# clberube/BISIP

Measured on AMD Instinct MI355X. Metric: log-prob evals/sec (walker-steps/s), PolynomialDecomposition 32 freq fp64, higher is better.
Workload: dtype f64; 1 GPU; PolynomialDecomposition poly_deg=5 c_exp=1.0, 32 synthetic frequencies (S=64 taus), ndim 7, theta uniform in the prior box; walkers_per_gpu=16777216, global_walkers=16777216, parallelism=walker-sharded x1, no data-path collective, kernel=k_logprob_pd_reduced, variant=reduced

## Files before the change

bisip_amd/_hip.py:

```python

import ctypes
import importlib.util
import os
import sys

import numpy as np

_HERE = os.path.dirname(os.path.abspath(__file__))
LIB_PATH = os.path.join(_HERE, 'libbisip_hip.so')

MODEL_POLYDECOMP, MODEL_COLECOLE, MODEL_DIAS2000, MODEL_SHIN2015 = 0, 1, 2, 3
VARIANT_AUTO, VARIANT_FAITHFUL, VARIANT_COLLAPSED, VARIANT_REDUCED, VARIANT_WAVE, VARIANT_REDUCED_COMP = 0, 1, 2, 3, 4, 5
VARIANTS = {'auto': VARIANT_AUTO, 'faithful': VARIANT_FAITHFUL, 'collapsed': VARIANT_COLLAPSED,
            'reduced': VARIANT_REDUCED, 'wave': VARIANT_WAVE, 'reduced_comp': VARIANT_REDUCED_COMP}

_dp = ctypes.POINTER(ctypes.c_double)


class ModelDesc(ctypes.Structure):
    _fields_ = [('n_modes', ctypes.c_int), ('poly_deg', ctypes.c_int), ('n_taus', ctypes.c_int),
                ('c_exp', ctypes.c_double), ('taus', _dp), ('log_taus', _dp)]


class StretchArgs(ctypes.Structure):
# ... 25 lines not shown
                                          ctypes.POINTER(ModelDesc)]),
    'bisip_ctx_nspectra': (ctypes.c_int, [ctypes.c_void_p]),
    'bisip_ctx_destroy': (None, [ctypes.c_void_p]),
    'bisip_ctx_set_bounds': (ctypes.c_int, [ctypes.c_void_p, _dp, _dp]),
    'bisip_ctx_set_spectrum_offset': (ctypes.c_int, [ctypes.c_void_p, ctypes.c_int64]),
    'bisip_ctx_set_variant': (ctypes.c_int, [ctypes.c_void_p, ctypes.c_int]),
    'bisip_ctx_get_variant': (ctypes.c_int, [ctypes.c_void_p]),
    'bisip_logprob': (ctypes.c_int, [ctypes.c_void_p, _dp, ctypes.c_int64, _dp]),
    'bisip_logprob_dev': (ctypes.c_int, [ctypes.c_void_p, ctypes.c_void_p, ctypes.c_int64,
                                         ctypes.c_void_p, ctypes.c_void_p]),
    'bisip_forward': (ctypes.c_int, [ctypes.c_void_p, _dp, ctypes.c_int64, _dp]),
    'bisip_forward_dev': (ctypes.c_int, [ctypes.c_void_p, ctypes.c_void_p, ctypes.c_int64,
                                         ctypes.c_void_p, ctypes.c_void_p]),
    'bisip_loglike_z': (ctypes.c_int, [ctypes.c_void_p, _dp, ctypes.c_int64, _dp]),
    'bisip_loglike_z_dev': (ctypes.c_int, [ctypes.c_void_p, ctypes.c_void_p, ctypes.c_int64,
                                           ctypes.c_void_p, ctypes.c_void_p]),
    'bisip_stretch_half_dev': (ctypes.c_int, [ctypes.c_void_p, ctypes.POINTER(StretchArgs), ctypes.c_void_p]),
    'bisip_stretch_eval_dev': (ctypes.c_int, [ctypes.c_void_p, ctypes.POINTER(StretchArgs), ctypes.c_void_p]),
    'bisip_stretch_apply_dev': (ctypes.c_int, [ctypes.c_void_p, ctypes.POINTER(StretchArgs), ctypes.c_void_p]),
    'bisip_stretch_run_dev': (ctypes.c_int, [ctypes.c_void_p, ctypes.POINTER(StretchArgs), ctypes.c_int64,
                                             ctypes.c_int64, ctypes.c_int64, ctypes.c_void_p]),
    'bisip_stretch_run_sharded_dev': (ctypes.c_int, [ctypes.c_void_p, ctypes.c_void_p, ctypes.POINTER(StretchArgs),
                                                     ctypes.c_int64, ctypes.c_int64, ctypes.c_int64, ctypes.c_void_p]),
    'bisip_stretch_run_sharded_sim_dev': (ctypes.c_int, [ctypes.c_void_p, ctypes.c_int, ctypes.POINTER(StretchArgs),
                                                         ctypes.c_int64, ctypes.c_int64, ctypes.c_int64, ctypes.c_void_p]),
    'bisip_rccl_unique_id': (ctypes.c_int, [ctypes.c_void_p]),
    'bisip_rccl_comm_create': (ctypes.c_int, [ctypes.POINTER(ctypes.c_void_p), ctypes.c_int, ctypes.c_int,
                                              ctypes.c_void_p, ctypes.c_int]),
    'bisip_rccl_comm_destroy': (ctypes.c_int, [ctypes.c_void_p]),
    'bisip_stretch_draw_dev': (ctypes.c_int, [ctypes.c_void_p, ctypes.c_int64, ctypes.c_double,
                                              ctypes.c_uint64, ctypes.c_int64, ctypes.c_int64] +
                               [ctypes.c_void_p] * 7),
    'bisip_stretch_philox_inline': (ctypes.c_int, [ctypes.c_void_p, ctypes.c_int64]),
    'bisip_stretch_run_philox_dev': (ctypes.c_int, [ctypes.c_void_p, ctypes.POINTER(StretchArgs), ctypes.c_int64, ctypes.c_int64,
                                                    ctypes.c_int64, ctypes.c_double, ctypes.c_uint64, ctypes.c_int64,
                                                    ctypes.c_void_p, ctypes.c_void_p]),
    'bisip_stretch_persistent_dev': (ctypes.c_int, [ctypes.c_void_p, ctypes.POINTER(PersistArgs), ctypes.c_void_p]),
    'bisip_chain_moments_workspace': (ctypes.c_int64, [ctypes.c_int64, ctypes.c_int64, ctypes.c_int]),
    'bisip_chain_moments_dev': (ctypes.c_int, [ctypes.c_void_p, ctypes.c_int64, ctypes.c_int64, ctypes.c_int64,
                                               ctypes.c_int64, ctypes.c_int] + [ctypes.c_void_p] * 4),
    'bisip_chain_percentiles_workspace': (ctypes.c_int64, [ctypes.c_int64, ctypes.c_int64, ctypes.c_int64, ctypes.c_int,
                                                           ctypes.c_int]),
    'bisip_chain_percentiles_dev': (ctypes.c_int, [ctypes.c_void_p, ctypes.c_int64, ctypes.c_int64, ctypes.c_int64,
                                                   ctypes.c_int64, ctypes.c_int, _dp, ctypes.c_int, ctypes.c_void_p,
                                                   ctypes.c_void_p, ctypes.c_int64, ctypes.c_void_p]),
    'bisip_chain_autocorr_time_workspace': (ctypes.c_int64, [ctypes.c_int64, ctypes.c_int64, ctypes.c_int64, ctypes.c_int]),
    'bisip_chain_autocorr_time_dev': (ctypes.c_int, [ctypes.c_void_p, ctypes.c_int64, ctypes.c_int64, ctypes.c_int64,
                                                     ctypes.c_int64, ctypes.c_int, ctypes.c_double] + [ctypes.c_void_p] * 4),
    'bisip_rtd_integrals_dev': (ctypes.c_int, [ctypes.c_void_p, ctypes.c_int64, ctypes.c_int64, ctypes.c_int64,
                                               ctypes.c_int64, ctypes.c_int] + [ctypes.c_void_p] * 4),
    'bisip_rtd_columns_dev': (ctypes.c_int, [ctypes.c_void_p, ctypes.c_int64, ctypes.c_int64, ctypes.c_int64,
                                             ctypes.c_int64, ctypes.c_int, ctypes.c_int64, ctypes.c_int64,
                                             ctypes.c_void_p, ctypes.c_int, ctypes.c_void_p, ctypes.c_void_p]),
    'bisip_chain_range_dev': (ctypes.c_int, [ctypes.c_void_p, ctypes.c_int64, ctypes.c_int64, ctypes.c_int64,
                                             ctypes.c_int64, ctypes.c_int] + [ctypes.c_void_p] * 3),
    'bisip_chain_histograms_dev': (ctypes.c_int, [ctypes.c_void_p, ctypes.c_int64, ctypes.c_int64, ctypes.c_int64,
                                                  ctypes.c_int64, ctypes.c_int, ctypes.c_void_p, ctypes.c_int,
                                                  ctypes.c_void_p, ctypes.c_void_p]),
    'bisip_chain_pair_histograms_dev': (ctypes.c_int, [ctypes.c_void_p, ctypes.c_int64, ctypes.c_int64, ctypes.c_int64,
                                                       ctypes.c_int64, ctypes.c_int, ctypes.c_void_p, ctypes.c_int,
                                                       ctypes.c_void_p, ctypes.c_void_p]),
    'bisip_chain_trace_workspace': (ctypes.c_int64, [ctypes.c_int64, ctypes.c_int64, ctypes.c_int64, ctypes.c_int, ctypes.c_int]),
    'bisip_chain_trace_lds_walkers': (ctypes.c_int, [ctypes.c_int]),
    'bisip_chain_trace_dev': (ctypes.c_int, [ctypes.c_void_p, ctypes.c_int64, ctypes.c_int64, ctypes.c_int64, ctypes.c_int64,
                                             ctypes.c_int, _dp, ctypes.c_int, ctypes.c_void_p, ctypes.c_void_p, ctypes.c_void_p,
                                             ctypes.c_int64, ctypes.c_void_p]),
# ... 419 lines not shown
                                                   int(W), ctypes.c_void_p(d_Z_ptr), ctypes.c_void_p(stream)))

    def stretch_half_dev(self, args, stream=0):
        _check(self._lib.bisip_stretch_half_dev(self._h, ctypes.byref(args), ctypes.c_void_p(stream)))

    def stretch_eval_dev(self, args, stream=0):
        _check(self._lib.bisip_stretch_eval_dev(self._h, ctypes.byref(args), ctypes.c_void_p(stream)))

    def stretch_apply_dev(self, args, stream=0):
        _check(self._lib.bisip_stretch_apply_dev(self._h, ctypes.byref(args), ctypes.c_void_p(stream)))

    def stretch_run_dev(self, first_args, W, n_steps, thin_by=1, stream=0):
        _check(self._lib.bisip_stretch_run_dev(self._h, ctypes.byref(first_args), int(W),
                                               int(n_steps), int(thin_by), ctypes.c_void_p(stream)))

    def stretch_run_sharded_dev(self, comm, first_args, W, n_steps, thin_by=1, stream=0):
        _check(self._lib.bisip_stretch_run_sharded_dev(self._h, ctypes.c_void_p(comm), ctypes.byref(first_args),
                                                       int(W), int(n_steps), int(thin_by), ctypes.c_void_p(stream)))

    def stretch_run_sharded_sim_dev(self, world, first_args, W, n_steps, thin_by=1, stream=0):
        _check(self._lib.bisip_stretch_run_sharded_sim_dev(self._h, int(world), ctypes.byref(first_args),
                                                           int(W), int(n_steps), int(thin_by), ctypes.c_void_p(stream)))

    def stretch_persistent_dev(self, args, stream=0):
        rc = self._lib.bisip_stretch_persistent_dev(self._h, ctypes.byref(args), ctypes.c_void_p(stream))
        if rc == -4:
            return False
        _check(rc)
        return True

    def stretch_philox_inline(self, W):
        return bool(self._lib.bisip_stretch_philox_inline(self._h, int(W)))

    def stretch_run_philox_dev(self, first_args, W, n_steps, thin_by, a, seed, step0, perm, stream=0):
        _check(self._lib.bisip_stretch_run_philox_dev(self._h, ctypes.byref(first_args), int(W), int(n_steps), int(thin_by),
                                                      float(a), int(seed), int(step0), ctypes.c_void_p(perm),
                                                      ctypes.c_void_p(stream)))

    def stretch_draw_dev(self, W, a, seed, step0, n_steps, perm, active, partner, zz, factor, logu,
                         stream=0):
        _check(self._lib.bisip_stretch_draw_dev(self._h, int(W), float(a), int(seed), int(step0),
                                                int(n_steps), *[ctypes.c_void_p(p) for p in
                                                                (perm, active, partner, zz, factor, logu)],
                                                ctypes.c_void_p(stream)))


RCCL_ID_BYTES = 128


def clock_probe_dev(d_out_ptr, window_us, stream=0):
    _check(load_library().bisip_clock_probe_dev(ctypes.c_void_p(d_out_ptr), float(window_us), ctypes.c_void_p(stream)))


def fp64_stream_probe_lanes():
    return int(load_library().bisip_fp64_stream_probe_lanes())


def fp64_stream_probe_dev(d_out_ptr, rounds, stream=0):
    n = ctypes.c_int64(0)
    _check(load_library().bisip_fp64_stream_probe_dev(ctypes.c_void_p(d_out_ptr), int(rounds), ctypes.byref(n), ctypes.c_void_p(stream)))
    return int(n.value)


def rccl_unique_id():
    buf = ctypes.create_string_buffer(RCCL_ID_BYTES)
    _check(load_library().bisip_rccl_unique_id(buf))
# ... 229 lines not shown
```

bisip_amd/csrc/bisip_hip.hip:

```cpp
#include <cstdlib>

#include "host.h"
#include "host_precompute.h"
#include "chain_kernels.h"

#include <atomic>
#include <exception>

using namespace bisip;
using namespace bisip::host;

namespace {
thread_local char g_err[512] = "";
}

namespace bisip {
namespace host {

int fail(int code, const char *fmt, ...)
{
    va_list ap;
    va_start(ap, fmt);
    vsnprintf(g_err, sizeof(g_err), fmt, ap);
    va_end(ap);
// ... 903 lines not shown
}

int bisip_stretch_eval_dev(bisip_ctx *c, const bisip_stretch_args *u, void *stream)
{
    int rc = check_stretch(c, u, true);
    if (rc != BISIP_OK || u->n_slots == 0) return rc;
    if (!u->partner || !u->zz || !u->factor || !u->logu) return fail(BISIP_EINVAL, "null RNG stream");
    if (u->slot_lo < 0 || u->slot_hi > u->n_slots || u->slot_lo > u->slot_hi)
        return fail(BISIP_EINVAL, "bad slot range [%lld,%lld) of %lld", (long long)u->slot_lo,
                    (long long)u->slot_hi, (long long)u->n_slots);
    if (u->slot_lo == u->slot_hi) return BISIP_OK;
    HIP_TRY(hipSetDevice(c->device));
    const StretchArgs a = to_device_args(u);
    return dispatch_stretch(c, StretchWork{STRETCH_EVAL, &a, nullptr}, u->walkers_per_spectrum, (hipStream_t)stream);
}

int bisip_stretch_apply_dev(bisip_ctx *c, const bisip_stretch_args *u, void *stream)
{
    int rc = check_stretch(c, u, true);
    if (rc != BISIP_OK || u->n_slots == 0) return rc;
    if (u->world < 1 || u->pad * u->world < u->n_slots)
        return fail(BISIP_EINVAL, "gathered block too small: world=%d pad=%lld n_slots=%lld", u->world,
                    (long long)u->pad, (long long)u->n_slots);
    HIP_TRY(hipSetDevice(c->device));
    return dispatch_apply(c, to_device_args(u), (hipStream_t)stream);
}

static bool packed_state(const bisip_ctx *c, int64_t W, int64_t n_steps)
{
    return c->E == 1 && c->ndim < PACKED_ROW && W / 2 >= 65536 && lanes_per_walker(W / 2) == 1 && n_steps > 0 &&
           std::getenv("BISIP_NO_PACKED_STATE") == nullptr;
}

struct PhiloxStream {
    double a;
    uint64_t seed;
    int64_t step0;
    const int32_t *d_perm;
};

static int stretch_run(bisip_ctx *c, const bisip_stretch_args *first, int64_t W, int64_t n_steps, int64_t thin_by,
                       const PhiloxStream *draw, void *stream)
{
    const int64_t nh = (W + 1) / 2;
    bisip_stretch_args u = *first;
    const bool packed = packed_state(c, W, n_steps);
    if (draw && !packed) return fail(BISIP_EUNSUPPORTED, "the stream is drawn in place only by the packed-state half-step (bisip_stretch_philox_inline)");
    if (packed) {
        const size_t need = (size_t)W * PACKED_ROW * sizeof(double);
        if (c->packed_bytes < need) {
            if (c->d_packed) { HIP_TRY(hipDeviceSynchronize()); (void)hipFree(c->d_packed); c->d_packed = nullptr; c->packed_bytes = 0; }
            hipError_t e = hipMalloc((void **)&c->d_packed, need);
            if (e != hipSuccess) return fail(BISIP_ENOMEM, "hipMalloc(%zu) failed: %s", need, hipGetErrorString(e));
            c->packed_bytes = need;
        }
        hipLaunchKernelGGL(k_state_repack<true>, dim3((unsigned)((W + 255) / 256)), dim3(256), 0, (hipStream_t)stream,
                           first->coords, first->logp, c->d_packed, (long long)W, c->ndim);
        HIP_TRY(hipGetLastError());
    }
    for (int64_t k = 0; k < n_steps; ++k) {
        for (int h = 0; h < 2; ++h) {
            const int64_t off = (k * 2 + h) * nh;
            if (!draw) {
                u.active = first->active + off; u.partner = first->partner + off;
                u.zz = first->zz + off; u.factor = first->factor + off; u.logu = first->logu + off;
            }
            u.n_slots = h ? W / 2 : nh;
            const bool store = ((k + 1) % thin_by) == 0;
            const int64_t srow = k / thin_by;
            u.chain_row = (store && first->chain_row) ? first->chain_row + srow * W * c->ndim : nullptr;
            u.logp_row = (store && first->logp_row) ? first->logp_row + srow * W : nullptr;
            StretchArgs a = to_device_args(&u);
            if (packed) a.packed = c->d_packed;
            if (draw) {
                a.perm = draw->d_perm + 3 * k;
                a.draw_W = W; a.draw_a = draw->a; a.draw_ndim_m1 = (double)(c->ndim - 1);
                a.seed_lo = (unsigned int)(draw->seed & 0xffffffffu); a.seed_hi = (unsigned int)(draw->seed >> 32);
                a.draw_step = (unsigned int)(draw->step0 + k); a.draw_e = (unsigned int)c->spectrum_offset; a.draw_h = h;
            }
            int rc = dispatch_stretch(c, StretchWork{STRETCH_HALF, &a, nullptr}, u.walkers_per_spectrum, (hipStream_t)stream);
            if (rc != BISIP_OK) return rc;
        }
    }
    if (packed) {
        hipLaunchKernelGGL(k_state_repack<false>, dim3((unsigned)((W + 255) / 256)), dim3(256), 0, (hipStream_t)stream,
                           first->coords, first->logp, c->d_packed, (long long)W, c->ndim);
        HIP_TRY(hipGetLastError());
    }
    return BISIP_OK;
}

int bisip_stretch_run_dev(bisip_ctx *c, const bisip_stretch_args *first, int64_t W, int64_t n_steps,
                          int64_t thin_by, void *stream)
{
    if (!c || !first) return fail(BISIP_EINVAL, "null argument");
    if (thin_by < 1 || n_steps % thin_by) return fail(BISIP_EINVAL, "n_steps=%lld must be a multiple of thin_by=%lld", (long long)n_steps, (long long)thin_by);
    if (W < 2 || n_steps < 0) return fail(BISIP_EINVAL, "bad W=%lld or n_steps=%lld", (long long)W, (long long)n_steps);
    if (!first->coords || !first->logp || !first->active || !first->partner || !first->zz ||
        !first->factor || !first->logu || !first->status)
        return fail(BISIP_EINVAL, "null buffer");
    HIP_TRY(hipSetDevice(c->device));
    return stretch_run(c, first, W, n_steps, thin_by, nullptr, stream);
}

int bisip_stretch_philox_inline(const bisip_ctx *c, int64_t W)
{
    return c && W >= 2 && W <= 0x7fffffffLL && packed_state(c, W, 1) ? 1 : 0;
}

int bisip_stretch_run_philox_dev(bisip_ctx *c, const bisip_stretch_args *first, int64_t W, int64_t n_steps,
                                 int64_t thin_by, double a, uint64_t seed, int64_t step0, const int32_t *d_perm,
                                 void *stream)
{
    if (!c || !first || !d_perm) return fail(BISIP_EINVAL, "null argument");
    if (thin_by < 1 || n_steps % thin_by) return fail(BISIP_EINVAL, "n_steps=%lld must be a multiple of thin_by=%lld", (long long)n_steps, (long long)thin_by);
    if (W < 2 || W > 0x7fffffffLL || n_steps < 0 || step0 < 0 || step0 + n_steps > 0xffffffffLL)
        return fail(BISIP_EINVAL, "bad W=%lld or step range [%lld, +%lld)", (long long)W, (long long)step0, (long long)n_steps);
    if (!(a > 0.0)) return fail(BISIP_EINVAL, "stretch scale a=%g must be positive", a);
    if (!first->coords || !first->logp || !first->status) return fail(BISIP_EINVAL, "null buffer");
    if (n_steps == 0) return BISIP_OK;
    HIP_TRY(hipSetDevice(c->device));
    const PhiloxStream draw{a, seed, step0, d_perm};
    return stretch_run(c, first, W, n_steps, thin_by, &draw, stream);
}

static double reduced_check_rows(const bisip_ctx *c, const double *theta, int64_t W, const double *logp,
                                 int64_t lo, int64_t hi, int64_t stride)
{
    constexpr int BLOCK = 64;
    const int64_t per = c->E > 1 ? W / c->E : W;
    const int n = c->ndim;
    double rows[BLOCK * MAXD], want[BLOCK], got[BLOCK];
    int held = 0;
    int64_t spectrum = -1;
    double w = 0.0;
    auto flush = [&] {
        if (!held) return;
        reduced_logp_reference_rows(c->reduced[(size_t)spectrum], rows, held, want);
        for (int r = 0; r < held; ++r) {
            const double scale = std::fabs(want[r]) > 1.0 ? std::fabs(want[r]) : 1.0;
// ... 361 lines not shown
```

bisip_amd/csrc/dispatch_stretch.hip:

```cpp
#include "stretch_launch.h"

using namespace bisip;
using namespace bisip::host;

namespace {

template <class M>
int stretch_generic(const bisip_ctx *c, const StretchWork &a, hipStream_t st)
{
    const ModelOperands o{c->d_cb_lp ? c->d_cb_lp : c->d_cb, c->N, c->lconst};
    if constexpr (CoopLimit<M>::value > 0) {
        switch (stretch_lanes(a)) {
        case 8: { GenericLP<M, 8> lp; lp.o = o; lp.b = c->bounds; return launch_stretch(a, lp, st); }
        case 4: { GenericLP<M, 4> lp; lp.o = o; lp.b = c->bounds; return launch_stretch(a, lp, st); }
        case 2: { GenericLP<M, 2> lp; lp.o = o; lp.b = c->bounds; return launch_stretch(a, lp, st); }
        default: break;
        }
    }
    GenericLP<M, 1> lp; lp.o = o; lp.b = c->bounds;
    return launch_stretch(a, lp, st);
}

template <int P, bool COMP>
int stretch_reduced(const bisip_ctx *c, const StretchWork &a, hipStream_t st)
{
    ReducedLP<P, COMP> lp;
    fill_reduced<P, COMP>(c, lp.r);
    lp.lconst = c->lconst;
    lp.b = c->bounds;
    return launch_stretch(a, lp, st);
}

}

namespace bisip {
namespace host {

StretchArgs to_device_args(const bisip_stretch_args *u)
{
    StretchArgs a;
    a.coords = u->coords; a.logp = u->logp;
    a.active = u->active; a.partner = u->partner;
    a.zz = u->zz; a.factor = u->factor; a.logu = u->logu;
    a.n_slots = u->n_slots; a.slot_lo = u->slot_lo; a.slot_hi = u->slot_hi;
    a.block = u->block; a.chain_row = u->chain_row; a.logp_row = u->logp_row;
    a.naccept = u->naccept; a.status = u->status;
    a.pad = u->pad;
    a.packed = nullptr;
    a.perm = nullptr; a.draw_W = 0; a.draw_a = 0.0; a.draw_ndim_m1 = 0.0;
    a.seed_lo = a.seed_hi = a.draw_step = a.draw_e = 0u; a.draw_h = 0;
    const long long world = u->world > 0 ? u->world : 1;
    a.base = u->n_slots / world;
    a.extra = u->n_slots % world;
    return a;
}

int dispatch_stretch(const bisip_ctx *c, const StretchWork &a, long long Wp, hipStream_t st)
{
    if (c->E > 1) {
        if (Wp < 2 || (Wp & 1)) return fail(BISIP_EINVAL, "batch context: walkers_per_spectrum must be even and >= 2, got %lld", Wp);
        return dispatch_stretch_batch(c, a, Wp, st);
    }
    switch (c->model_id) {
    case BISIP_MODEL_POLYDECOMP:
        if (effective_variant(c) == BISIP_VARIANT_FAITHFUL || effective_variant(c) == BISIP_VARIANT_WAVE)
            return fail(BISIP_EUNSUPPORTED, "the device stretch move has no kernel for the faithful / wave "
                        "formulation: use variant auto, reduced or collapsed, or the host-loop sampler");
        if (effective_variant(c) == BISIP_VARIANT_REDUCED) {
            switch (c->P) {
#define X(p) case p: return stretch_reduced<p, false>(c, a, st);
                PD_CASES(X)
#undef X
            }
        } else if (effective_variant(c) == BISIP_VARIANT_REDUCED_COMP) {
            switch (c->P) {
#define X(p) case p: return stretch_reduced<p, true>(c, a, st);
                PD_CASES(X)
#undef X
            }
        } else {
            switch (c->P) {
#define X(p) case p: return stretch_generic<PDCollapsed<p>>(c, a, st);
// ... 34 lines not shown
```

bisip_amd/csrc/sampler_kernels.h:

```cpp
#pragma once
#include <type_traits>
#include "kernels.h"
#include "philox.h"

namespace bisip {

struct StretchArgs {
    double *coords;
    double *logp;
    const int *active;
    const int *partner;
    const double *zz;
    const double *factor;
    const double *logu;
    long long n_slots;
    long long slot_lo, slot_hi;
    double *block;
    double *chain_row;
    double *logp_row;
    int *naccept;
    int *status;
    long long pad, base, extra;
    double *packed;
    const int *perm;
    long long draw_W;
    double draw_a, draw_ndim_m1;
    unsigned int seed_lo, seed_hi, draw_step, draw_e;
    int draw_h;
};

template <class LP, class = void>
struct MayPersist : std::true_type {};
template <class LP>
struct MayPersist<LP, std::void_t<decltype(LP::WAVE_IN_ONE_SPECTRUM)>> : std::bool_constant<LP::WAVE_IN_ONE_SPECTRUM> {};

template <class LP, class = void>
struct SingleSpectrum : std::false_type {};
template <class LP>
struct SingleSpectrum<LP, std::void_t<decltype(LP::SINGLE_SPECTRUM)>> : std::bool_constant<LP::SINGLE_SPECTRUM> {};

template <class M, int L_ = 1>
struct GenericLP {
    static constexpr bool SINGLE_SPECTRUM = true;
    static constexpr int NDIM = M::NDIM;
    static constexpr int L = L_;
    static constexpr bool CAN_STAGE = true;
    static constexpr int REC_DOUBLES = M::REC;
    ModelOperands o;
    Bounds b;
    __device__ __forceinline__ double operator()(const double (&th)[NDIM], int, int g) const
    {
        return logprob_row<M, L>(th, o, b, g);
    }
    __device__ __forceinline__ const double *records(long long) const { return o.cb; }
    __host__ __device__ __forceinline__ int n_freq() const { return o.N; }
    struct Local {};
    __device__ __forceinline__ Local local(long long) const { return {}; }
// ... 223 lines not shown
                        a.zz[t], a.factor[t], a.logu[t], lp, i, g, a.status, row, lp_row);
}

template <int NDIM>
__device__ __forceinline__ void commit_row(const StretchArgs &a, int i, const double (&row)[NDIM],
                                           double lp_row, bool acc)
{
    if (acc) {
#pragma unroll
        for (int k = 0; k < NDIM; ++k) a.coords[(long long)i * NDIM + k] = row[k];
        a.logp[i] = lp_row;
    }
    if (a.chain_row) {
#pragma unroll
        for (int k = 0; k < NDIM; ++k) a.chain_row[(long long)i * NDIM + k] = row[k];
    }
    if (a.logp_row) a.logp_row[i] = lp_row;
    if (a.naccept && acc) atomicAdd(a.naccept + i, 1);
}

__device__ __forceinline__ int perm_inverse(long long y, long long W, long long Ainv, long long B)
{
    long long v = y - B;
    if (v < 0) v += W;
    if (W <= 65536) return (int)(((unsigned)Ainv * (unsigned)v) % (unsigned)W);
    const unsigned long long prod = (unsigned long long)Ainv * (unsigned long long)v;
    const unsigned q = (unsigned)((double)prod * (1.0 / (double)W));
    long long r = (long long)(prod - (unsigned long long)q * (unsigned long long)W);
    if (r < 0) r += W;
    if (r >= W) r -= W;
    return (int)r;
}

struct SlotDraw {
    int active, partner;
    double z, factor, logu;
};

__device__ __forceinline__ SlotDraw draw_slot(long long W, double a, double ndim_m1, unsigned seed_lo,
                                              unsigned seed_hi, unsigned step, int h, unsigned e,
                                              long long t, long long A_inv, long long B)
{
    const long long Nc = h ? (W + 1) / 2 : W / 2;
    const unsigned c2 = (unsigned)h | (e << 1);
    const Philox4 r0 = philox4x32_10((unsigned)t, step, c2, 0u, seed_lo, seed_hi);
    const Philox4 r1 = philox4x32_10((unsigned)t, step, c2, 1u, seed_lo, seed_hi);
    const double uz = u53(r0.v[0], r0.v[1]);
    const long long r = (long long)(((unsigned long long)r0.v[2] * (unsigned long long)Nc) >> 32);
    const double v = (a - 1.0) * uz + 1.0;
    SlotDraw d;
    d.z = (v * v) / a;
    d.active = perm_inverse(2 * t + h, W, A_inv, B);
    d.partner = perm_inverse(2 * r + (1 - h), W, A_inv, B);
    d.factor = ndim_m1 * log(d.z);
    d.logu = log(u53(r1.v[0], r1.v[1]));
    return d;
}

template <class LP, int BLK = 64>
__global__ __launch_bounds__(BLK) void k_stretch_half(const StretchArgs a, const LP lp)
{
    constexpr int L = LP::L;
    const long long tid = (long long)blockIdx.x * BLK + threadIdx.x;
    const long long slot = tid / L;
    const int g = (int)(tid % L);
    const bool live = slot < a.n_slots;
    const long long t = live ? slot : a.n_slots - 1;
    int i;
    double row[LP::NDIM], lp_row;
    const bool acc = stretch_slot(a, lp, t, g, i, row, lp_row);
    if (live && g == 0) commit_row<LP::NDIM>(a, i, row, lp_row, acc);
}

constexpr int PACKED_ROW = 8;

template <class LP, int BLK = 256>
__global__ __launch_bounds__(BLK) void k_stretch_half_packed(const StretchArgs a, const LP lp)
{
    static_assert(LP::L == 1 && LP::NDIM < PACKED_ROW, "one lane per slot, a walker in one 64-byte row");
    constexpr int NDIM = LP::NDIM;
    const long long slot = (long long)blockIdx.x * BLK + threadIdx.x;
    const bool live = slot < a.n_slots;
    const long long t = live ? slot : a.n_slots - 1;
    int i, p;
    double z, factor, logu;
    if (a.perm) {
        const SlotDraw d = draw_slot(a.draw_W, a.draw_a, a.draw_ndim_m1, a.seed_lo, a.seed_hi, a.draw_step, a.draw_h,
                                     a.draw_e, t, a.perm[1], a.perm[2]);
        i = d.active; p = d.partner; z = d.z; factor = d.factor; logu = d.logu;
    } else {
        i = __builtin_nontemporal_load(a.active + t); p = __builtin_nontemporal_load(a.partner + t);
    }
    const dbl2 *srow = reinterpret_cast<const dbl2 *>(a.packed + (long long)i * PACKED_ROW);
    const dbl2 *crow = reinterpret_cast<const dbl2 *>(a.packed + (long long)p * PACKED_ROW);
    dbl2 sv[4], cv[4];
#pragma unroll
    for (int q = 0; q < 4; ++q) { sv[q] = srow[q]; cv[q] = crow[q]; }
    if (!a.perm) {
        z = __builtin_nontemporal_load(a.zz + t); factor = __builtin_nontemporal_load(a.factor + t);
        logu = __builtin_nontemporal_load(a.logu + t);
    }
    double s_row[PACKED_ROW], c_row[PACKED_ROW];
#pragma unroll
    for (int q = 0; q < 4; ++q) { s_row[2 * q] = sv[q].x; s_row[2 * q + 1] = sv[q].y; c_row[2 * q] = cv[q].x; c_row[2 * q + 1] = cv[q].y; }
    double row[NDIM], lp_row;
    const bool acc = stretch_move(s_row, c_row, s_row[PACKED_ROW - 1], z, factor, logu, lp, i, 0, a.status, row, lp_row);
    if (!live) return;
    if (acc) {
        double r[PACKED_ROW];
#pragma unroll
        for (int q = 0; q < PACKED_ROW; ++q) r[q] = q < NDIM ? row[q] : 0.0;
        r[PACKED_ROW - 1] = lp_row;
        dbl2 *dst = reinterpret_cast<dbl2 *>(a.packed + (long long)i * PACKED_ROW);
#pragma unroll
        for (int q = 0; q < 4; ++q) { dbl2 v; v.x = r[2 * q]; v.y = r[2 * q + 1]; dst[q] = v; }
        if (a.naccept) atomicAdd(a.naccept + i, 1);
    }
    if (a.chain_row) {
#pragma unroll
        for (int k = 0; k < NDIM; ++k) __builtin_nontemporal_store(row[k], a.chain_row + (long long)i * NDIM + k);
    }
    if (a.logp_row) __builtin_nontemporal_store(lp_row, a.logp_row + i);
}

template <bool PACK>
__global__ __launch_bounds__(256) void k_state_repack(double *coords, double *logp, double *packed, long long W, int ndim)
{
    __shared__ __attribute__((aligned(16))) double tile[256 * PACKED_ROW];
    const long long row0 = (long long)blockIdx.x * 256;
    const int rows = (int)(W - row0 < 256 ? W - row0 : 256);
    const int tid = threadIdx.x;
    dbl2 *tile2 = reinterpret_cast<dbl2 *>(tile);
    dbl2 *packed2 = reinterpret_cast<dbl2 *>(packed + row0 * PACKED_ROW);
    if (PACK) {
        for (int idx = tid; idx < rows * ndim; idx += 256) {
            const int w = idx / ndim, q = idx - w * ndim;
            tile[w * PACKED_ROW + q] = coords[row0 * ndim + idx];
        }
        if (tid < rows) {
            for (int q = ndim; q < PACKED_ROW - 1; ++q) tile[tid * PACKED_ROW + q] = 0.0;
            tile[tid * PACKED_ROW + PACKED_ROW - 1] = logp[row0 + tid];
        }
        __syncthreads();
        for (int j = tid; j < rows * (PACKED_ROW / 2); j += 256) packed2[j] = tile2[j];
    } else {
        for (int j = tid; j < rows * (PACKED_ROW / 2); j += 256) tile2[j] = packed2[j];
        __syncthreads();
        for (int idx = tid; idx < rows * ndim; idx += 256) {
            const int w = idx / ndim, q = idx - w * ndim;
            coords[row0 * ndim + idx] = tile[w * PACKED_ROW + q];
        }
        if (tid < rows) logp[row0 + tid] = tile[tid * PACKED_ROW + PACKED_ROW - 1];
    }
}


template <class LP>
__global__ __launch_bounds__(64) void k_stretch_eval(const StretchArgs a, const LP lp)
{
    constexpr int NDIM = LP::NDIM;
    constexpr int L = LP::L;
    const long long tid = (long long)blockIdx.x * 64 + threadIdx.x;
    const long long slot = a.slot_lo + tid / L;
    const int g = (int)(tid % L);
    const bool live = slot < a.slot_hi;
    const long long t = live ? slot : a.slot_hi - 1;
    int i;
    double row[NDIM], lp_row;
    const bool acc = stretch_slot(a, lp, t, g, i, row, lp_row);
    if (!live || g != 0) return;
    double *out = a.block + (t - a.slot_lo) * (NDIM + 2);
#pragma unroll
    for (int k = 0; k < NDIM; ++k) out[k] = row[k];
    out[NDIM] = lp_row;
    out[NDIM + 1] = acc ? 1.0 : 0.0;
}

template <int NDIM>
__global__ __launch_bounds__(64) void k_stretch_apply(const StretchArgs a)
{
    const long long t = (long long)blockIdx.x * 64 + threadIdx.x;
    if (t >= a.n_slots) return;
    long long r, off;
    const long long big = a.extra * (a.base + 1);
    if (t < big) { r = t / (a.base + 1); off = t - r * (a.base + 1); }
// ... 361 lines not shown
```

bisip_amd/csrc/stretch_launch.h:

```cpp
#pragma once
#include "host.h"

#include <cstdlib>

namespace bisip {
namespace host {

template <class LP>
int launch_persistent(const PersistArgs &p0, const LP &lp, hipStream_t st)
{
    PersistArgs p = p0;
    const long long nh = (p.W + 1) / 2;
    p.lanes_per_ens = (int)(((nh * LP::L + 63) / 64) * 64);
    const size_t state_bytes = (size_t)p.W * (LP::NDIM + 1) * sizeof(double);
    size_t rec_bytes = 0;
    if constexpr (LP::CAN_STAGE) {
        const bool off = std::getenv("BISIP_NO_LDS_STAGING") != nullptr;
        rec_bytes = off ? 0 : (((size_t)lp.n_freq() * LP::REC_DOUBLES + 1) & ~(size_t)1) * sizeof(double);
        if (state_bytes + rec_bytes + 16 > 65536) rec_bytes = 0;
    }
    p.rec_stride = (long long)(rec_bytes / sizeof(double));
    long long epw = 1;
    if (p.E > 1) {
        epw = 256 / p.lanes_per_ens;
// ... 36 lines not shown
        }
        p.spread = p.G > 32 ? 1 : 0;
        const dim3 grid((unsigned)(p.spread ? p.G : 8 * p.G)), block(BLK);
        if constexpr (LP::CAN_STAGE) {
            if (rec_bytes) {
                hipLaunchKernelGGL((k_stretch_group<LP, true, BLK>), grid, block, rec_bytes, st, p, lp);
                HIP_TRY(hipGetLastError());
                return BISIP_OK;
            }
        }
        hipLaunchKernelGGL((k_stretch_group<LP, false, BLK>), grid, block, 0, st, p, lp);
        HIP_TRY(hipGetLastError());
        return BISIP_OK;
    }
}

template <class LP>
int launch_stretch(const StretchWork &work, const LP &lp, hipStream_t st)
{
    const StretchKind kind = work.kind;
    if constexpr (LP::L == 8) {
        if (kind != STRETCH_GROUP) return fail(BISIP_EUNSUPPORTED, "internal: eight lanes per slot outside the multi-workgroup sampler");
        return launch_group(*work.persist, lp, st);
    } else {
    if (kind == STRETCH_PERSIST) {
        if constexpr (MayPersist<LP>::value) return launch_persistent(*work.persist, lp, st);
        else return fail(BISIP_EUNSUPPORTED, "internal: a persistent launch for a functor whose waves straddle spectra");
    }
    if (kind == STRETCH_GROUP) return launch_group(*work.persist, lp, st);
    const StretchArgs &a = *work.half;
    if (kind == STRETCH_HALF) {
        if (a.packed) {
            if constexpr (LP::L == 1 && LP::NDIM < PACKED_ROW && SingleSpectrum<LP>::value) {
                const unsigned grid = (unsigned)((a.n_slots + 255) / 256);
                hipLaunchKernelGGL((k_stretch_half_packed<LP, 256>), dim3(grid), dim3(256), 0, st, a, lp);
            } else {
                return fail(BISIP_EUNSUPPORTED, "internal: a packed state for a kernel that has no packed form");
            }
        } else if (a.n_slots * LP::L >= 65536) {
            const unsigned grid = (unsigned)((a.n_slots * LP::L + 255) / 256);
            hipLaunchKernelGGL((k_stretch_half<LP, 256>), dim3(grid), dim3(256), 0, st, a, lp);
        } else {
            const unsigned grid = (unsigned)((a.n_slots * LP::L + 63) / 64);
            hipLaunchKernelGGL((k_stretch_half<LP, 64>), dim3(grid), dim3(64), 0, st, a, lp);
        }
    } else {
        if constexpr (SingleSpectrum<LP>::value) {
            const unsigned grid = (unsigned)(((a.slot_hi - a.slot_lo) * LP::L + 63) / 64);
            hipLaunchKernelGGL((k_stretch_eval<LP>), dim3(grid), dim3(64), 0, st, a, lp);
        } else {
            return fail(BISIP_EUNSUPPORTED, "the sharded half-step takes a single-spectrum context");
        }
    }
    HIP_TRY(hipGetLastError());
    return BISIP_OK;
    }
}

inline int stretch_lanes(const StretchWork &w)
{
    if (const char *env = std::getenv("BISIP_STRETCH_LANES")) {
        const int v = std::atoi(env);
        if (w.kind == STRETCH_GROUP && (v == 1 || v == 2 || v == 4 || v == 8)) return v;
        if (v == 1 || v == 2 || v == 4) {
            if (w.kind != STRETCH_PERSIST) return v;
            const long long nh = (w.persist->W + 1) / 2;
            return nh * v <= 512 ? v : (nh * 2 <= 512 ? 2 : 1);
        }
// ... 20 lines not shown
```

bisip_amd/sampler.py:

```python

import os

import numpy as np

from .chainview import _DeviceSlabs, _merge_device_parts
from .dist import all_gather_rows, shard_range
from .summaries import DeviceChainSummaries


class _one_blas_thread(object):

    _lock = None
    _controller = None
    _n_libs = -1

    def __enter__(self):
        import threading
        cls = _one_blas_thread
        if cls._lock is None:
            cls._lock = threading.Lock()
        self._ctx = None
        cls._lock.acquire()
        try:
            import sys
# ... 535 lines not shown
        if ev is not None:
            ev.synchronize()
        out = {}
        for name, dt in kinds:
            blk = _pinned_scratch(f'{self._key}stream_{slot}_{name}', need * 8)
            out[name] = blk[:need * (4 if dt == torch.int32 else 8)].view(dt).view(int(n), 2, int(nh))
        return out

    def upload_staged(self, stage, slot=0):
        out = {name: t.to(self.device, non_blocking=True) for name, t in stage.items()}
        ev = self.torch.cuda.Event()
        ev.record(self.torch.cuda.current_stream(self.device))
        _PINNED[f'{self._key}stream_event_{slot}'] = ev
        return out

    def host_buffer(self, shape):
        nbytes = 8 * int(np.prod(shape))
        return self.torch.empty(shape, dtype=self.torch.float64, pin_memory=nbytes >= (32 << 20))

    def copy_out(self, dst_host, src_dev):
        torch = self.torch
        if not hasattr(self, '_copy_stream'):
            self._copy_stream = torch.cuda.Stream(self.device)
        ev = torch.cuda.Event()
        ev.record(torch.cuda.current_stream(self.device))
        self._copy_stream.wait_event(ev)
        with torch.cuda.stream(self._copy_stream):
            dst_host.copy_(src_dev, non_blocking=True)
        src_dev.record_stream(self._copy_stream)

    def draws_in_place(self, W):
        import os
        return os.environ.get('BISIP_NO_INLINE_DRAW') is None and self.ctx.stretch_philox_inline(W)

    def draw(self, st, W, a, seed, step0, n_steps, after=None):
        stream = self.stream()
        if after is not None:
            torch = self.torch
            if not hasattr(self, '_draw_stream'):
                self._draw_stream = torch.cuda.Stream(self.device)
            for ev in after:
                if ev is not None:
                    self._draw_stream.wait_event(ev)
            stream = self._draw_stream.cuda_stream
        self.ctx.stretch_draw_dev(W, a, seed, step0, n_steps, st['perm'].data_ptr(),
                                  st['active'].data_ptr(), st['partner'].data_ptr(),
                                  st['zz'].data_ptr(), st['factor'].data_ptr(),
                                  st['logu'].data_ptr(), stream)
        if after is not None:
            done = self.torch.cuda.Event()
            done.record(self._draw_stream)
            self.torch.cuda.current_stream(self.device).wait_event(done)

    def mark(self):
        ev = self.torch.cuda.Event()
        ev.record(self.torch.cuda.current_stream(self.device))
        return ev

    def synchronize(self):
        self.torch.cuda.synchronize(self.device)


class DeviceEnsembleSampler(DeviceChainSummaries, _SamplerBase):

    def __init__(self, nwalkers, ndim, ctx=None, a=2.0, live_dangerously=False, group=None,
                 distributed=False, backend=None, chunk=None, rng='numpy', seed=None,
# ... 5 lines not shown
        self.walkers_per_ensemble = int(nwalkers)
        if self.n_ensembles > 1:
            if rng != 'philox':
                raise ValueError("n_ensembles > 1 needs rng='philox'")
            if nwalkers % 2:
                raise ValueError('n_ensembles > 1 needs an even number of walkers per ensemble')
            if distributed:
                raise ValueError('independent ensembles shard as whole replicas; run one sampler per rank')
        self.backend = backend if backend is not None else HipStretchBackend(ctx)
        self.chunk = chunk
        self.rng = rng
        self.force_sharded_path = bool(force_sharded_path)
        self.simulate_world = 0
        if isinstance(sharded_loop, str) and sharded_loop.startswith('simulate:'):
            self.simulate_world = int(sharded_loop.split(':', 1)[1])
            if self.simulate_world < 1 or distributed:
                raise ValueError("sharded_loop='simulate:N' needs N >= 1 and a single process")
            sharded_loop = 'python'
            self.force_sharded_path = True
        if sharded_loop not in ('rccl', 'rccl-own', 'python'):
            raise ValueError("sharded_loop must be 'rccl', 'rccl-own', 'python' or 'simulate:N'")
        self.sharded_loop = sharded_loop
        self._comm, self._comm_owned, self._comm_tried = None, False, False
        if persistent is None:
            ctx = getattr(self.backend, 'ctx', None)
            limit = getattr(ctx, 'persistent_walkers', 128)
            if int(nwalkers) * self.n_ensembles >= 65536 and self.n_ensembles > 1:
                persistent = limit > 0 and int(nwalkers) <= 1024 and getattr(ctx, 'persistent_in_big_batches', True)
            else:
                persistent = int(nwalkers) <= limit or (self.n_ensembles == 1 and 1024 < int(nwalkers) <= getattr(ctx, 'group_walkers', 0))
        self.persistent = bool(persistent)
        self.chain_on_device = bool(chain_on_device)
        self.last_path = None
        self.last_stream = None
        super().__init__(int(nwalkers) * self.n_ensembles, ndim, a, live_dangerously, group, distributed)
        self.seed = None
        if rng == 'philox':
            self.seed = int(seed) if seed is not None else int(self._random.randint(0, 2 ** 31 - 1))
        self._dev = None
        self._iterations_run = 0

    def reset(self):
        super().reset()
        dev = getattr(self, '_dev', None)
        if dev is not None:
            dev['naccept'].zero_()
        self._accepted_before = np.zeros(self.nwalkers)

    def _sharded_comm(self):
        if self._comm is None and not self._comm_tried:
            self._comm_tried = True
            if hasattr(self.backend, 'rccl_comm') and self.sharded_loop != 'python':
                self._comm, self._comm_owned = self.backend.rccl_comm(
                    self._group, self._world, self._rank,
                    prefer='own' if self.sharded_loop == 'rccl-own' else 'torch', in_group=self._in_group)
        return self._comm

    def close(self):
        if getattr(self, '_comm', None) is not None and self._comm_owned:
            from . import _hip
            self.backend.synchronize()
            _hip.rccl_comm_destroy(self._comm)
        self._comm, self._comm_owned = None, False

    def __del__(self):
        try:
# ... 145 lines not shown
                        dist.all_gather_into_tensor(host, block.cpu(), group=self._group)
                        gathered.copy_(host)
                    else:
                        dist.all_gather_into_tensor(gathered, block, group=self._group)
                    be.apply(st, k, h, m, gathered, pad, self._world)

    def run_mcmc(self, initial_state, nsteps, progress=False, thin_by=1, **kwargs):
        import time
        import torch
        t_start = time.perf_counter()
        be = self.backend
        W, ndim = self.nwalkers, self.ndim
        setup_detail = self._start_from(initial_state)
        nsteps, thin_by = int(nsteps), int(thin_by)
        if thin_by < 1:
            raise ValueError('thin_by must be >= 1')
        nh = (W + 1) // 2
        chain_host = logp_host = None
        dev_chain = dev_logp = None
        stream_bufs = [None, None]
        free_ev = [None, None]
        perm_ev = None
        perm_all = None
        if self.rng == 'philox' and nsteps > 0:
            perm_all = be.tensor(affine_splits(self.seed, self.walkers_per_ensemble,
                                               self._iterations_run, nsteps * thin_by), slot='c')
            perm_ev = be.mark() if hasattr(be, 'mark') else None
        self.timing = dict(setup_s=time.perf_counter() - t_start, stream_s=0.0, enqueue_s=0.0, alloc_s=0.0,
                           drain_s=0.0, finish_s=0.0, **setup_detail)
        it_start = self._iterations_run
        in_place = (self.rng == 'philox' and self.n_ensembles == 1 and self._world == 1 and not self.force_sharded_path
                    and not self.simulate_world and hasattr(be, 'draws_in_place') and be.draws_in_place(W))
        self.last_stream = 'in place' if in_place else ('arrays' if self.rng == 'philox' else 'host')
        sizes, left = [], nsteps
        while left > 0:
            sizes.append(min(max(1, self._chunk_steps(nsteps * thin_by, in_place) // thin_by), left))
            left -= sizes[-1]
        if not in_place and self.rng == 'philox' and sizes:
            need = 2 * sizes[0] * thin_by * 2 * nh * 32
            if need > (32 << 30):
                import warnings
                warnings.warn(f'thin_by={thin_by} with {W} walkers needs {need / 2**30:.0f} GiB of random-stream arrays per chunk '
                              '(a chunk holds whole thinning intervals); consider a smaller thin_by', ResourceWarning, stacklevel=2)
        first_sample = [0]
        for ns in sizes:
            first_sample.append(first_sample[-1] + ns)
        ahead = None
        rng_state0 = self._random.get_state() if self.rng == 'numpy' else None
        nan_initial = False
        guard = self._guard_plan()
        self.guard_ = dict(checks=0, rows=0, worst=0.0, escalations=0, reruns=0, kernel=None)
        saved = {}
        final = {}
        E, Wp = self.n_ensembles, self.walkers_per_ensemble

        def enqueue(k):
            nonlocal ahead, dev_chain, dev_logp, chain_host, logp_host, perm_ev, nan_initial
            t_a = time.perf_counter()
            ns = sizes[k]
            n = ns * thin_by
            done, it0 = first_sample[k], it_start + first_sample[k] * thin_by
            rec = dict(k=k, ns=ns)
            st = dict(self._dev)
            st['nh'] = nh
            st['thin'] = thin_by
            if self.n_ensembles > 1:
# ... 202 lines not shown
```

include/bisip_hip.h:

```cpp
#ifndef BISIP_HIP_H
#define BISIP_HIP_H

#include <stdint.h>

#ifdef __cplusplus
extern "C" {
#endif

#define BISIP_ABI_VERSION 6

#define BISIP_MODEL_POLYDECOMP 0
#define BISIP_MODEL_COLECOLE   1
#define BISIP_MODEL_DIAS2000   2
#define BISIP_MODEL_SHIN2015   3

#define BISIP_VARIANT_AUTO      0
#define BISIP_VARIANT_FAITHFUL  1
#define BISIP_VARIANT_COLLAPSED 2
#define BISIP_VARIANT_REDUCED   3
#define BISIP_VARIANT_WAVE      4
#define BISIP_VARIANT_REDUCED_COMP 5

#define BISIP_OK          0
#define BISIP_EINVAL     -1
// ... 69 lines not shown
    int32_t *naccept;
    int32_t *status;
    int64_t pad;
    int32_t world;
    int64_t walkers_per_spectrum;
} bisip_stretch_args;

int bisip_stretch_half_dev(bisip_ctx *ctx, const bisip_stretch_args *args, void *stream);
int bisip_stretch_eval_dev(bisip_ctx *ctx, const bisip_stretch_args *args, void *stream);
int bisip_stretch_apply_dev(bisip_ctx *ctx, const bisip_stretch_args *args, void *stream);

int bisip_stretch_run_dev(bisip_ctx *ctx, const bisip_stretch_args *first, int64_t W,
                          int64_t n_steps, int64_t thin_by, void *stream);

int bisip_stretch_run_sharded_dev(bisip_ctx *ctx, void *comm, const bisip_stretch_args *first,
                                  int64_t W, int64_t n_steps, int64_t thin_by, void *stream);

int bisip_stretch_run_sharded_sim_dev(bisip_ctx *ctx, int world, const bisip_stretch_args *first, int64_t W,
                                      int64_t n_steps, int64_t thin_by, void *stream);

#define BISIP_RCCL_ID_BYTES 128
int bisip_rccl_unique_id(void *id);
int bisip_rccl_comm_create(void **comm, int world, int rank, const void *id, int device);
int bisip_rccl_comm_destroy(void *comm);

int bisip_ctx_set_spectrum_offset(bisip_ctx *ctx, int64_t first_spectrum);

int bisip_stretch_draw_dev(bisip_ctx *ctx, int64_t W, double a, uint64_t seed, int64_t step0,
                           int64_t n_steps, const int32_t *d_perm, int32_t *d_active,
                           int32_t *d_partner, double *d_zz, double *d_factor, double *d_logu,
                           void *stream);

int bisip_stretch_philox_inline(const bisip_ctx *ctx, int64_t W);
int bisip_stretch_run_philox_dev(bisip_ctx *ctx, const bisip_stretch_args *first, int64_t W, int64_t n_steps,
                                 int64_t thin_by, double a, uint64_t seed, int64_t step0, const int32_t *d_perm,
                                 void *stream);

typedef struct bisip_persist_args {
    double *coords;
    double *logp;
    int64_t n_walkers;
    int64_t walkers_per_ensemble;
    int64_t n_steps;
    int64_t thin_by;
    const int32_t *active;
    const int32_t *partner;
    const double *zz;
    const double *factor;
    const double *logu;
    double *chain;
    double *logp_chain;
    int32_t *naccept;
    int32_t *status;
} bisip_persist_args;
int bisip_stretch_persistent_dev(bisip_ctx *ctx, const bisip_persist_args *args, void *stream);

int64_t bisip_chain_moments_workspace(int64_t n_samples, int64_t n_ensembles, int ndim);
int bisip_chain_moments_dev(const double *d_chain, int64_t n_samples, int64_t sample_stride,
                            int64_t n_ensembles, int64_t walkers_per_ensemble, int ndim,
                            double *d_mean, double *d_std, double *d_work, void *stream);

int64_t bisip_chain_percentiles_workspace(int64_t n_samples, int64_t n_ensembles,
                                          int64_t walkers_per_ensemble, int ndim, int n_percentiles);
int bisip_chain_percentiles_dev(const double *d_chain, int64_t n_samples, int64_t sample_stride,
                                int64_t n_ensembles, int64_t walkers_per_ensemble, int ndim,
                                const double *percentiles, int n_percentiles, double *d_out,
// ... 126 lines not shown
```

Measured before the change: 100.6 billion evals/s.

## Walk the packed half-step in walker order with a parity-split state layout

```diff
diff --git a/bisip_amd/_hip.py b/bisip_amd/_hip.py
--- a/bisip_amd/_hip.py
+++ b/bisip_amd/_hip.py
@@ -81,6 +81,7 @@
                                               ctypes.c_uint64, ctypes.c_int64, ctypes.c_int64] +
                                [ctypes.c_void_p] * 7),
     'bisip_stretch_philox_inline': (ctypes.c_int, [ctypes.c_void_p, ctypes.c_int64]),
+    'bisip_stretch_walker_order': (ctypes.c_int, [ctypes.c_void_p, ctypes.c_int64]),
     'bisip_stretch_run_philox_dev': (ctypes.c_int, [ctypes.c_void_p, ctypes.POINTER(StretchArgs), ctypes.c_int64, ctypes.c_int64,
                                                     ctypes.c_int64, ctypes.c_double, ctypes.c_uint64, ctypes.c_int64,
                                                     ctypes.c_void_p, ctypes.c_void_p]),
@@ -566,6 +567,9 @@
     def stretch_philox_inline(self, W):
         return bool(self._lib.bisip_stretch_philox_inline(self._h, int(W)))
 
+    def stretch_walker_order(self, W):
+        return bool(self._lib.bisip_stretch_walker_order(self._h, int(W)))
+
     def stretch_run_philox_dev(self, first_args, W, n_steps, thin_by, a, seed, step0, perm, stream=0):
         _check(self._lib.bisip_stretch_run_philox_dev(self._h, ctypes.byref(first_args), int(W), int(n_steps), int(thin_by),
                                                       float(a), int(seed), int(step0), ctypes.c_void_p(perm),
diff --git a/bisip_amd/csrc/bisip_hip.hip b/bisip_amd/csrc/bisip_hip.hip
--- a/bisip_amd/csrc/bisip_hip.hip
+++ b/bisip_amd/csrc/bisip_hip.hip
@@ -959,6 +959,11 @@
            std::getenv("BISIP_NO_PACKED_STATE") == nullptr;
 }
 
+static bool walker_order(int64_t W)
+{
+    return (W & 1) == 0 && std::getenv("BISIP_NO_WALKER_ORDER") == nullptr;
+}
+
 struct PhiloxStream {
     double a;
     uint64_t seed;
@@ -973,6 +978,7 @@
     bisip_stretch_args u = *first;
     const bool packed = packed_state(c, W, n_steps);
     if (draw && !packed) return fail(BISIP_EUNSUPPORTED, "the stream is drawn in place only by the packed-state half-step (bisip_stretch_philox_inline)");
+    const bool in_walker_order = packed && draw && walker_order(W);
     if (packed) {
         const size_t need = (size_t)W * PACKED_ROW * sizeof(double);
         if (c->packed_bytes < need) {
@@ -981,7 +987,8 @@
             if (e != hipSuccess) return fail(BISIP_ENOMEM, "hipMalloc(%zu) failed: %s", need, hipGetErrorString(e));
             c->packed_bytes = need;
         }
-        hipLaunchKernelGGL(k_state_repack<true>, dim3((unsigned)((W + 255) / 256)), dim3(256), 0, (hipStream_t)stream,
+        hipLaunchKernelGGL((in_walker_order ? k_state_repack<true, true> : k_state_repack<true, false>),
+                           dim3((unsigned)((W + 255) / 256)), dim3(256), 0, (hipStream_t)stream,
                            first->coords, first->logp, c->d_packed, (long long)W, c->ndim);
         HIP_TRY(hipGetLastError());
     }
@@ -1001,6 +1008,7 @@
             if (packed) a.packed = c->d_packed;
             if (draw) {
                 a.perm = draw->d_perm + 3 * k;
+                a.walker_order = in_walker_order ? 1 : 0;
                 a.draw_W = W; a.draw_a = draw->a; a.draw_ndim_m1 = (double)(c->ndim - 1);
                 a.seed_lo = (unsigned int)(draw->seed & 0xffffffffu); a.seed_hi = (unsigned int)(draw->seed >> 32);
                 a.draw_step = (unsigned int)(draw->step0 + k); a.draw_e = (unsigned int)c->spectrum_offset; a.draw_h = h;
@@ -1010,7 +1018,8 @@
         }
     }
     if (packed) {
-        hipLaunchKernelGGL(k_state_repack<false>, dim3((unsigned)((W + 255) / 256)), dim3(256), 0, (hipStream_t)stream,
+        hipLaunchKernelGGL((in_walker_order ? k_state_repack<false, true> : k_state_repack<false, false>),
+                           dim3((unsigned)((W + 255) / 256)), dim3(256), 0, (hipStream_t)stream,
                            first->coords, first->logp, c->d_packed, (long long)W, c->ndim);
         HIP_TRY(hipGetLastError());
     }
@@ -1033,6 +1042,11 @@
 int bisip_stretch_philox_inline(const bisip_ctx *c, int64_t W)
 {
     return c && W >= 2 && W <= 0x7fffffffLL && packed_state(c, W, 1) ? 1 : 0;
+}
+
+int bisip_stretch_walker_order(const bisip_ctx *c, int64_t W)
+{
+    return bisip_stretch_philox_inline(c, W) && walker_order(W) ? 1 : 0;
 }
 
 int bisip_stretch_run_philox_dev(bisip_ctx *c, const bisip_stretch_args *first, int64_t W, int64_t n_steps,
diff --git a/bisip_amd/csrc/dispatch_stretch.hip b/bisip_amd/csrc/dispatch_stretch.hip
--- a/bisip_amd/csrc/dispatch_stretch.hip
+++ b/bisip_amd/csrc/dispatch_stretch.hip
@@ -47,7 +47,7 @@
     a.naccept = u->naccept; a.status = u->status;
     a.pad = u->pad;
     a.packed = nullptr;
-    a.perm = nullptr; a.draw_W = 0; a.draw_a = 0.0; a.draw_ndim_m1 = 0.0;
+    a.perm = nullptr; a.walker_order = 0; a.draw_W = 0; a.draw_a = 0.0; a.draw_ndim_m1 = 0.0;
     a.seed_lo = a.seed_hi = a.draw_step = a.draw_e = 0u; a.draw_h = 0;
     const long long world = u->world > 0 ? u->world : 1;
     a.base = u->n_slots / world;
diff --git a/bisip_amd/csrc/sampler_kernels.h b/bisip_amd/csrc/sampler_kernels.h
--- a/bisip_amd/csrc/sampler_kernels.h
+++ b/bisip_amd/csrc/sampler_kernels.h
@@ -23,6 +23,7 @@
     long long pad, base, extra;
     double *packed;
     const int *perm;
+    int walker_order;
     long long draw_W;
     double draw_a, draw_ndim_m1;
     unsigned int seed_lo, seed_hi, draw_step, draw_e;
@@ -312,11 +313,22 @@
     return (int)r;
 }
 
+__device__ __forceinline__ long long perm_forward(long long i, long long W, long long A, long long B)
+{
+    const unsigned long long prod = (unsigned long long)A * (unsigned long long)i + (unsigned long long)B;
+    const unsigned q = (unsigned)((double)prod * (1.0 / (double)W));
+    long long r = (long long)(prod - (unsigned long long)q * (unsigned long long)W);
+    if (r < 0) r += W;
+    if (r >= W) r -= W;
+    return r;
+}
+
 struct SlotDraw {
     int active, partner;
     double z, factor, logu;
 };
 
+template <bool ACTIVE = true>
 __device__ __forceinline__ SlotDraw draw_slot(long long W, double a, double ndim_m1, unsigned seed_lo,
                                               unsigned seed_hi, unsigned step, int h, unsigned e,
                                               long long t, long long A_inv, long long B)
@@ -330,7 +342,7 @@
     const double v = (a - 1.0) * uz + 1.0;
     SlotDraw d;
     d.z = (v * v) / a;
-    d.active = perm_inverse(2 * t + h, W, A_inv, B);
+    d.active = ACTIVE ? perm_inverse(2 * t + h, W, A_inv, B) : -1;
     d.partner = perm_inverse(2 * r + (1 - h), W, A_inv, B);
     d.factor = ndim_m1 * log(d.z);
     d.logu = log(u53(r1.v[0], r1.v[1]));
@@ -353,6 +365,27 @@
 }
 
 constexpr int PACKED_ROW = 8;
+
+template <int NDIM>
+__device__ __forceinline__ void packed_commit(const StretchArgs &a, int i, long long at, const double (&row)[NDIM],
+                                              double lp_row, bool acc)
+{
+    if (acc) {
+        double r[PACKED_ROW];
+#pragma unroll
+        for (int q = 0; q < PACKED_ROW; ++q) r[q] = q < NDIM ? row[q] : 0.0;
+        r[PACKED_ROW - 1] = lp_row;
+        dbl2 *dst = reinterpret_cast<dbl2 *>(a.packed + at * PACKED_ROW);
+#pragma unroll
+        for (int q = 0; q < 4; ++q) { dbl2 v; v.x = r[2 * q]; v.y = r[2 * q + 1]; dst[q] = v; }
+        if (a.naccept) atomicAdd(a.naccept + i, 1);
+    }
+    if (a.chain_row) {
+#pragma unroll
+        for (int k = 0; k < NDIM; ++k) __builtin_nontemporal_store(row[k], a.chain_row + (long long)i * NDIM + k);
+    }
+    if (a.logp_row) __builtin_nontemporal_store(lp_row, a.logp_row + i);
+}
 
 template <class LP, int BLK = 256>
 __global__ __launch_bounds__(BLK) void k_stretch_half_packed(const StretchArgs a, const LP lp)
@@ -385,25 +418,39 @@
     for (int q = 0; q < 4; ++q) { s_row[2 * q] = sv[q].x; s_row[2 * q + 1] = sv[q].y; c_row[2 * q] = cv[q].x; c_row[2 * q + 1] = cv[q].y; }
     double row[NDIM], lp_row;
     const bool acc = stretch_move(s_row, c_row, s_row[PACKED_ROW - 1], z, factor, logu, lp, i, 0, a.status, row, lp_row);
-    if (!live) return;
-    if (acc) {
-        double r[PACKED_ROW];
-#pragma unroll
-        for (int q = 0; q < PACKED_ROW; ++q) r[q] = q < NDIM ? row[q] : 0.0;
-        r[PACKED_ROW - 1] = lp_row;
-        dbl2 *dst = reinterpret_cast<dbl2 *>(a.packed + (long long)i * PACKED_ROW);
-#pragma unroll
-        for (int q = 0; q < 4; ++q) { dbl2 v; v.x = r[2 * q]; v.y = r[2 * q + 1]; dst[q] = v; }
-        if (a.naccept) atomicAdd(a.naccept + i, 1);
-    }
-    if (a.chain_row) {
-#pragma unroll
-        for (int k = 0; k < NDIM; ++k) __builtin_nontemporal_store(row[k], a.chain_row + (long long)i * NDIM + k);
-    }
-    if (a.logp_row) __builtin_nontemporal_store(lp_row, a.logp_row + i);
-}
-
-template <bool PACK>
+    if (live) packed_commit<NDIM>(a, i, i, row, lp_row, acc);
+}
+
+template <class LP, int BLK = 256>
+__global__ __launch_bounds__(BLK) void k_stretch_half_walker_order(const StretchArgs a, const LP lp)
+{
+    static_assert(LP::L == 1 && LP::NDIM < PACKED_ROW, "one lane per walker, a walker in one 64-byte row");
+    constexpr int NDIM = LP::NDIM;
+    const long long W = a.draw_W, half = W >> 1;
+    const long long lane = (long long)blockIdx.x * BLK + threadIdx.x;
+    const bool live = lane < half;
+    const long long j = live ? lane : half - 1;
+    const long long B = a.perm[2];
+    const int par = (int)((a.draw_h ^ B) & 1);
+    const int i = (int)(2 * j + par);
+    const long long t = perm_forward(i, W, a.perm[0], B) >> 1;
+    const SlotDraw d = draw_slot<false>(W, a.draw_a, a.draw_ndim_m1, a.seed_lo, a.seed_hi, a.draw_step, a.draw_h,
+                                        a.draw_e, t, a.perm[1], B);
+    const long long own = par * half + j, other = (1 - par) * half + (d.partner >> 1);
+    const dbl2 *srow = reinterpret_cast<const dbl2 *>(a.packed + own * PACKED_ROW);
+    const dbl2 *crow = reinterpret_cast<const dbl2 *>(a.packed + other * PACKED_ROW);
+    dbl2 sv[4], cv[4];
+#pragma unroll
+    for (int q = 0; q < 4; ++q) { sv[q] = srow[q]; cv[q] = crow[q]; }
+    double s_row[PACKED_ROW], c_row[PACKED_ROW];
+#pragma unroll
+    for (int q = 0; q < 4; ++q) { s_row[2 * q] = sv[q].x; s_row[2 * q + 1] = sv[q].y; c_row[2 * q] = cv[q].x; c_row[2 * q + 1] = cv[q].y; }
+    double row[NDIM], lp_row;
+    const bool acc = stretch_move(s_row, c_row, s_row[PACKED_ROW - 1], d.z, d.factor, d.logu, lp, i, 0, a.status, row, lp_row);
+    if (live) packed_commit<NDIM>(a, i, own, row, lp_row, acc);
+}
+
+template <bool PACK, bool SPLIT = false>
 __global__ __launch_bounds__(256) void k_state_repack(double *coords, double *logp, double *packed, long long W, int ndim)
 {
     __shared__ __attribute__((aligned(16))) double tile[256 * PACKED_ROW];
@@ -411,26 +458,38 @@
     const int rows = (int)(W - row0 < 256 ? W - row0 : 256);
     const int tid = threadIdx.x;
     dbl2 *tile2 = reinterpret_cast<dbl2 *>(tile);
-    dbl2 *packed2 = reinterpret_cast<dbl2 *>(packed + row0 * PACKED_ROW);
+    dbl2 *packed2 = reinterpret_cast<dbl2 *>(packed);
+    auto tile_row = [](int w) { return SPLIT ? (w & 1) * 128 + (w >> 1) : w; };
+    auto packed_row = [&](int r) -> long long {
+        if (!SPLIT) return r < rows ? row0 + r : -1;
+        const int odd = r >> 7, k = r & 127;
+        return k < ((rows + 1 - odd) >> 1) ? odd * (W >> 1) + (row0 >> 1) + k : -1;
+    };
     if (PACK) {
         for (int idx = tid; idx < rows * ndim; idx += 256) {
             const int w = idx / ndim, q = idx - w * ndim;
-            tile[w * PACKED_ROW + q] = coords[row0 * ndim + idx];
+            tile[tile_row(w) * PACKED_ROW + q] = coords[row0 * ndim + idx];
         }
         if (tid < rows) {
-            for (int q = ndim; q < PACKED_ROW - 1; ++q) tile[tid * PACKED_ROW + q] = 0.0;
-            tile[tid * PACKED_ROW + PACKED_ROW - 1] = logp[row0 + tid];
+            for (int q = ndim; q < PACKED_ROW - 1; ++q) tile[tile_row(tid) * PACKED_ROW + q] = 0.0;
+            tile[tile_row(tid) * PACKED_ROW + PACKED_ROW - 1] = logp[row0 + tid];
         }
         __syncthreads();
-        for (int j = tid; j < rows * (PACKED_ROW / 2); j += 256) packed2[j] = tile2[j];
+        for (int j = tid; j < 256 * (PACKED_ROW / 2); j += 256) {
+            const long long at = packed_row(j >> 2);
+            if (at >= 0) packed2[at * (PACKED_ROW / 2) + (j & 3)] = tile2[j];
+        }
     } else {
-        for (int j = tid; j < rows * (PACKED_ROW / 2); j += 256) tile2[j] = packed2[j];
+        for (int j = tid; j < 256 * (PACKED_ROW / 2); j += 256) {
+            const long long at = packed_row(j >> 2);
+            if (at >= 0) tile2[j] = packed2[at * (PACKED_ROW / 2) + (j & 3)];
+        }
         __syncthreads();
         for (int idx = tid; idx < rows * ndim; idx += 256) {
             const int w = idx / ndim, q = idx - w * ndim;
-            coords[row0 * ndim + idx] = tile[w * PACKED_ROW + q];
-        }
-        if (tid < rows) logp[row0 + tid] = tile[tid * PACKED_ROW + PACKED_ROW - 1];
+            coords[row0 * ndim + idx] = tile[tile_row(w) * PACKED_ROW + q];
+        }
+        if (tid < rows) logp[row0 + tid] = tile[tile_row(tid) * PACKED_ROW + PACKED_ROW - 1];
     }
 }
 
diff --git a/bisip_amd/csrc/stretch_launch.h b/bisip_amd/csrc/stretch_launch.h
--- a/bisip_amd/csrc/stretch_launch.h
+++ b/bisip_amd/csrc/stretch_launch.h
@@ -92,8 +92,13 @@
     if (kind == STRETCH_HALF) {
         if (a.packed) {
             if constexpr (LP::L == 1 && LP::NDIM < PACKED_ROW && SingleSpectrum<LP>::value) {
-                const unsigned grid = (unsigned)((a.n_slots + 255) / 256);
-                hipLaunchKernelGGL((k_stretch_half_packed<LP, 256>), dim3(grid), dim3(256), 0, st, a, lp);
+                if (a.walker_order) {
+                    const unsigned grid = (unsigned)((a.draw_W / 2 + 255) / 256);
+                    hipLaunchKernelGGL((k_stretch_half_walker_order<LP, 256>), dim3(grid), dim3(256), 0, st, a, lp);
+                } else {
+                    const unsigned grid = (unsigned)((a.n_slots + 255) / 256);
+                    hipLaunchKernelGGL((k_stretch_half_packed<LP, 256>), dim3(grid), dim3(256), 0, st, a, lp);
+                }
             } else {
                 return fail(BISIP_EUNSUPPORTED, "internal: a packed state for a kernel that has no packed form");
             }
diff --git a/bisip_amd/sampler.py b/bisip_amd/sampler.py
--- a/bisip_amd/sampler.py
+++ b/bisip_amd/sampler.py
@@ -591,6 +591,9 @@
     def draws_in_place(self, W):
         import os
         return os.environ.get('BISIP_NO_INLINE_DRAW') is None and self.ctx.stretch_philox_inline(W)
+
+    def walks_in_walker_order(self, W):
+        return self.ctx.stretch_walker_order(W)
 
     def draw(self, st, W, a, seed, step0, n_steps, after=None):
         stream = self.stream()
@@ -662,6 +665,7 @@
         self.persistent = bool(persistent)
         self.chain_on_device = bool(chain_on_device)
         self.last_path = None
+        self.last_order = None
         self.last_stream = None
         super().__init__(int(nwalkers) * self.n_ensembles, ndim, a, live_dangerously, group, distributed)
         self.seed = None
@@ -873,6 +877,7 @@
         in_place = (self.rng == 'philox' and self.n_ensembles == 1 and self._world == 1 and not self.force_sharded_path
                     and not self.simulate_world and hasattr(be, 'draws_in_place') and be.draws_in_place(W))
         self.last_stream = 'in place' if in_place else ('arrays' if self.rng == 'philox' else 'host')
+        self.last_order = 'walker' if in_place and be.walks_in_walker_order(W) else 'slot'
         sizes, left = [], nsteps
         while left > 0:
             sizes.append(min(max(1, self._chunk_steps(nsteps * thin_by, in_place) // thin_by), left))
diff --git a/include/bisip_hip.h b/include/bisip_hip.h
--- a/include/bisip_hip.h
+++ b/include/bisip_hip.h
@@ -125,6 +125,7 @@
                            void *stream);
 
 int bisip_stretch_philox_inline(const bisip_ctx *ctx, int64_t W);
+int bisip_stretch_walker_order(const bisip_ctx *ctx, int64_t W);
 int bisip_stretch_run_philox_dev(bisip_ctx *ctx, const bisip_stretch_args *first, int64_t W, int64_t n_steps,
                                  int64_t thin_by, double a, uint64_t seed, int64_t step0, const int32_t *d_perm,
                                  void *stream);
```

Measured after the change: 101.2 billion evals/s, median of 2. No clear change (+0.6%).
